# zichunhao/lgn-autoencoder

Measured on AMD Instinct MI355X. Metric: jets/sec fwd+bwd, 30-particle maxdim=2 bs=512, higher is better.
Workload: dtype f64

## Files before the change

### lgn-autoencoder_amd/csrc/level.hpp

```cpp
#pragma once
#include "common.hpp"

namespace lgn {

constexpr int LVL_DEC_PAIRWISE = 2;
constexpr int LVL_LEVEL_V2 = 4;
constexpr int LVL_MLP_V1 = 8;
constexpr int LVL_MOMENTS_V1 = 16;
constexpr int LVL_MLP_BWD1 = 1024;
constexpr int LVL_MLP_FULLTILE = 2048;
constexpr int LVL_MOMENTS_SPLIT = 512;
constexpr int LVL_LIVE_SCALARS = 4096;
constexpr int LVL_BWD_ORDERED = 64;
int level_flags_from_env();

template <typename T>
struct LevelArgs {
  int B, N, C, CO;
  const T* s_in;
  const T* v_in;
  const T* p;
  const uint8_t* mask;
  const T *ra, *rb, *rc, *w0, *b0, *w1, *b1;
  const T *wm0, *wm1;
  T* ag0;
  T* ag1;
  T* s_out;
// ... 5 lines not shown
  T* z1 = nullptr;
  size_t z1n = 0;
  T* z2 = nullptr;
  size_t z2n = 0;
  const T* loss_wo1 = nullptr;
  const T* loss_target = nullptr;
  T loss_scale = T(1);
  int loss_real = 0;
  T loss_jscale = T(0);
  T* loss_recon = nullptr;
  T* loss_part = nullptr;
  T* loss_gv = nullptr;
  T* loss_wpart = nullptr;
  int flags = 0;
  int dead_scalars = 0;
};

template <typename T>
struct LevelBwdArgs {
  int B, N, C, CO;
  const T *s_in, *v_in, *p;
  const uint8_t* mask;
  const T *ra, *rb, *rc, *w0, *b0, *w1, *b1;
  const T *wm0, *wm1;
  const T *ag0, *ag1;
  const T* g_s_out;
  const T* g_v_out;
  T* g_ag;
  T* g_s_in;
  T* g_v_in;
  T* g_p;
  T* part_mix;
  T* part_rad;
  T* part_in0 = nullptr;
  int flags = 0;
  int dead_scalars = 0;
};

__host__ __device__ constexpr int node_stride(int C) { return 10 * C + 4; }

__host__ __device__ constexpr int rad_partial_size(int C, bool dec) {
  return dec ? 2 * C : (2 * 4 * C * NB + 8 * C);
}

inline int level_jet_split(int B, int N) {
  const int groups = (N + 3) / 4;
  int s = 1;
  while (s * 2 <= groups && B * s * 2 <= 512) s *= 2;
  return s;
}

// ... 2 lines not shown
```

### lgn-autoencoder_amd/csrc/level_bwd.hip

```cpp
#include <stdlib.h>

#include "level_dev.hpp"
#include <type_traits>
#include "ops.hpp"
#include "tail_dev.hpp"

namespace lgn {

template <int C> struct GA {
  static constexpr int A3 = 0, A4 = 2 * C, A1 = 4 * C, A2 = 12 * C, SIZE = 20 * C;
};

template <typename T, int C>
__global__ __launch_bounds__(BLOCK) void level_bwd_mix_kernel(LevelBwdArgs<T> a) {
  constexpr int IT = 32;
  constexpr int K = 5 * C;
  constexpr int XS = K * 10;
  const int N = a.N, B = a.B, CO = a.CO;
  const int b = blockIdx.x, tile = blockIdx.y, tid = threadIdx.x;
  const int GS = CO * 10;

  extern __shared__ __align__(16) unsigned char smem_raw[];
  T* sm = reinterpret_cast<T*>(smem_raw);
  T* wm = sm;
// ... 340 lines not shown
  return 0;
}

int level_bwd_nodes2_dispatch(const LevelBwdArgs<double>& a, int decoder, hipStream_t stream);
int level_bwd_rad2_dispatch(const LevelBwdArgs<double>& a, hipStream_t stream);

int level_bwd3_dispatch(const LevelBwdArgs<double>& a, int decoder, hipStream_t stream);
int level_bwd_dec_sep_dispatch(const LevelBwdArgs<double>& a, hipStream_t stream);
int level_bwd_sweep_enc_dispatch(const LevelBwdArgs<double>& a, hipStream_t stream);
static bool dec_pairwise(int flags) { return (flags & LVL_DEC_PAIRWISE) != 0; }
bool level_bwd3_fits(int N);

static bool use_v3(int N, int flags) { return !(flags & LVL_LEVEL_V2) && level_bwd3_fits(N); }

bool level_bwd_carries_input(int N, int flags) { return use_v3(N, flags); }

void level_bwd_partial_rows(int B, int N, int decoder, int flags, int* rows_mix, int* rows_rad) {
  const int tiles = cdiv(N, 32);
  if (use_v3(N, flags)) {
    const int split = (decoder && !dec_pairwise(flags)) ? 1 : level_jet_split(B, N);
    *rows_mix = B * split;
    *rows_rad = B * split;
    return;
  }
  *rows_mix = B * tiles;
  if (decoder && dec_pairwise(flags)) {
    *rows_rad = B * tiles;
  } else {
    *rows_rad = B;
  }
}

template <typename T, int C, bool DEC>
static int launch_level_bwd(const LevelBwdArgs<T>& a, hipStream_t stream) {
  using L = Carve<C, DEC>;
  const int N = a.N, CO = a.CO, tiles = cdiv(N, 32);
  int rc;
  if (use_v3(N, a.flags)) return level_bwd3_dispatch(a, DEC, stream);
  {
    auto kern = level_bwd_mix_kernel<T, C>;
    size_t smem = sizeof(T) * (4 * CO * 5 * C + 32 * (5 * C * 10) + 32 * CO * 10);
    if ((rc = ensure_smem(kern, smem, "level_bwd_mix"))) return rc;
    hipLaunchKernelGGL(kern, dim3(a.B, tiles), dim3(BLOCK), smem, stream, a);
    LGN_CHECK_LAUNCH();
  }
  if constexpr (DEC && std::is_same<T, double>::value) {
    if (!dec_pairwise(a.flags)) return level_bwd_dec_sep_dispatch(a, stream);
  }
  if constexpr (!DEC && std::is_same<T, double>::value) {
    if (!(a.flags & LVL_LEVEL_V2)) return level_bwd_sweep_enc_dispatch(a, stream);
  }
  if ((rc = level_bwd_nodes2_dispatch(a, DEC, stream))) return rc;
  if (DEC) {
// ... 110 lines not shown
```

### lgn-autoencoder_amd/csrc/level_bwd3.hip

```cpp
#include "pair_dev.hpp"
#include "ops.hpp"
#include "wave_sum.hpp"

namespace lgn {

namespace {
LGN_STAMP_DECL
}
LGN_STAMP_READER(lgn_debug_stamps_bwd3)

template <int C, bool DEC, int NWV = 4>
struct Bwd3 {
  static constexpr int BLK = 64 * NWV;
  static constexpr int NG = (C + 3) / 4;
  static constexpr int NS = node_stride(C);
  static constexpr int PS = DEC ? 8 : 4;
  static constexpr int TRSZ = DEC ? NWV * 64 : NWV * pair_scratch(NG);
  static constexpr int MIXP = BLK / (5 * C) < 16 ? BLK / (5 * C) : 16;
  __host__ __device__ static size_t scratch(int N, int CO) {
    size_t p1 = (size_t)N * 10 * CO + 4 * CO * 5 * C + (size_t)N * 20 * C;
    const size_t red = (size_t)MIXP * CO * 5 * C * 4;
    if (red > p1) p1 = red;
    return p1 > (size_t)TRSZ ? p1 : (size_t)TRSZ;
  }
// ... 19 lines not shown
  const int nlo = min(N, 4 * glo), nhi = min(N, 4 * ghi);
  const size_t prow = (size_t)b * gridDim.y + blockIdx.y;

  extern __shared__ __align__(16) unsigned char smem_raw[];
  double* nd = reinterpret_cast<double*>(smem_raw);
  double* ga = nd + ((N * NS + 1) & ~1);
  double* gd = ga + N * G::SIZE;
  double* pj = gd + N * 10 * C;
  double* tr = pj + N * PS;
  double* go = tr;
  double* wm = go + N * 10 * CO;
  double* agl = wm + 4 * CO * K;
  double* sm = tr + F::scratch(N, CO);
  uint8_t* mk = reinterpret_cast<uint8_t*>(sm + F::SEPSZ);

  STAMP(0);
  {
    const size_t plo = (size_t)B * N * CO, pa = (size_t)B * N * 2 * C;
    JetRegs<double> jr;
    load_jet_issue<double, C, DEC>(a.s_in, a.v_in, a.p, a.mask, B, N, b, jr);
    const int eg = tid < N * CO ? tid : 0, ea_ = tid < N * 2 * C ? tid : 0, ew = tid < 2 * CO * K ? tid : 0;
    const size_t ig = (size_t)b * N * CO + eg, ia = (size_t)b * N * 2 * C + ea_;
    double rg[10], ra[10];
    if constexpr (!NOS) {
      rg[0] = a.g_s_out[ig];
      rg[1] = a.g_s_out[plo + ig];
      ra[0] = a.ag0[ia];
      ra[1] = a.ag0[pa + ia];
    }
#pragma unroll
    for (int m = 0; m < 4; ++m) {
      rg[2 + m] = a.g_v_out[ig * 4 + m];
      rg[6 + m] = a.g_v_out[plo * 4 + ig * 4 + m];
      ra[2 + m] = a.ag1[ia * 4 + m];
      ra[6 + m] = a.ag1[(pa + ia) * 4 + m];
    }
    const double w0v = a.wm0[ew], w1v = a.wm1[ew];
    load_jet_commit<double, C, DEC>(a.s_in, a.v_in, a.p, a.mask, B, N, b, jr, nd, pj, mk);
    if (tid < N * CO) {
#pragma unroll
      for (int m = NOS ? 2 : 0; m < 10; ++m) go[tid * 10 + m] = rg[m];
    }
    if (tid < N * 2 * C) {
#pragma unroll
      for (int m = NOS ? 2 : 0; m < 10; ++m) agl[tid * 10 + m] = ra[m];
    }
    if (tid < 2 * CO * K) {
      wm[tid] = w0v;
      wm[2 * CO * K + tid] = w1v;
    }
    for (int e = tid + BLK; e < 2 * CO * K; e += BLK) {
      wm[e] = a.wm0[e];
      wm[2 * CO * K + e] = a.wm1[e];
    }
    for (int e = tid + BLK; e < N * CO; e += BLK) {
      const size_t idx = (size_t)b * N * CO + e;
      double* g = go + e * 10;
      if constexpr (!NOS) {
        g[0] = a.g_s_out[idx];
        g[1] = a.g_s_out[plo + idx];
      }
#pragma unroll
      for (int m = 0; m < 4; ++m) {
        g[2 + m] = a.g_v_out[idx * 4 + m];
        g[6 + m] = a.g_v_out[plo * 4 + idx * 4 + m];
      }
    }
    for (int e = tid + BLK; e < N * 2 * C; e += BLK) {
      const size_t ea = (size_t)b * N * 2 * C + e;
      double* x = agl + e * 10;
      if constexpr (!NOS) {
        x[0] = a.ag0[ea];
        x[1] = a.ag0[pa + ea];
      }
#pragma unroll
      for (int m = 0; m < 4; ++m) {
        x[2 + m] = a.ag1[ea * 4 + m];
        x[6 + m] = a.ag1[(pa + ea) * 4 + m];
      }
    }
  }
  __syncthreads();
  STAMP(1);

  {
    const int half = tid >= BLK / 2;
    for (int e = half ? tid - BLK / 2 : tid; e < N * C; e += BLK / 2) {
      const int n = e / C, c = e - n * C;
      const double* w0r = wm + c;
      const double* w1r = wm + 2 * CO * K + c;
      if (half == 0) {
        cx<double> gx0[2] = {{0, 0}, {0, 0}}, gx1[2][4] = {{{0, 0}, {0, 0}, {0, 0}, {0, 0}}, {{0, 0}, {0, 0}, {0, 0}, {0, 0}}};
        for (int o = 0; o < CO; ++o) {
          const double* g = go + (n * CO + o) * 10;
          cx<double> gv[4];
#pragma unroll
          for (int m = 0; m < 4; ++m) gv[m] = {g[2 + m], g[6 + m]};
// ... 131 lines not shown
    STAMP(51);
    for (int ex = tid; ex < 4 * OK; ex += BLK) {
      const int e = ex >> 2, x = ex & 3;
      if (NOS && x < 2) continue;
      double v = red[ex];
#pragma unroll
      for (int pp = 1; pp < NPART; ++pp) v += red[pp * OK * 4 + ex];
      part[x * OK + e] = v;
    }
  }

  if constexpr (DEC && SEP) {
    STAMP(3);
    __syncthreads();
    STAMP(4);
    if (tid < 64) {
      const int k = tid & 7, part = tid >> 3;
      double mean = 0.0;
      for (int n = part; n < N; n += 8) mean += pj[n * 8 + k];
      mean += shfl_xor(mean, 8);
      mean += shfl_xor(mean, 16);
      mean += shfl_xor(mean, 32);
      if (part == 0) sm[k] = mean / N;
    }
    __syncthreads();
    for (int e = tid; e < N * 8; e += BLK) pj[e] -= sm[e & 7];
    __syncthreads();
#define LGN_PUT(k, val)                                       \
  do {                                                        \
    if ((k) < 16) a0[(k) < 16 ? (k) : 0] += (val);                                        \
    else if ((k) < 32) a1[(k) >= 16 && (k) < 32 ? (k) - 16 : 0] += (val);                 \
    else if ((k) < 44) a2[(k) >= 32 && (k) < 44 ? (k) - 32 : 0] += (val);                 \
    else a3[(k) >= 44 ? (k) - 44 : 0] += (val);                                           \
  } while (0)
    for (int c = wave; c < C; c += NWV) {
      double a0[16], a1[16], a2[12], a3[8];
#pragma unroll
      for (int k = 0; k < 16; ++k) a0[k] = a1[k] = 0.0;
#pragma unroll
      for (int k = 0; k < 12; ++k) a2[k] = 0.0;
#pragma unroll
      for (int k = 0; k < 8; ++k) a3[k] = 0.0;
// ... 529 lines not shown
    rad_rows_store(tr, wave, lane, T);
    __syncthreads();
    const int wq = __builtin_amdgcn_readfirstlane(wave);
    if (wq < 4) rad_rows_sum<C, NWV, WaveSum::Pairwise, true>(tr, part, lane, wq);
  }
  STAMP(10);
}

bool level_bwd3_fits(int N) { return N <= 40; }

template <int C, bool DEC, bool SEP, int NWV, bool NOS>
static int launch_bwd3_w(const LevelBwdArgs<double>& a, int split, hipStream_t stream) {
  size_t smem = Bwd3<C, DEC, NWV>::smem(a.N, a.CO);
  LGN_CHECK_ARG(smem <= 160 * 1024, "level_bwd: N=%d C=%d needs %zu B of LDS", a.N, a.C, smem);
  LGN_CHECK_ARG(a.CO <= 8, "level_bwd: C_out=%d unsupported (1..8)", a.CO);
  auto kern = level_bwd3_kernel<C, DEC, SEP, NWV, false, NOS>;
  if constexpr (!DEC && C <= 4) {
    if (split == 1 && !(a.flags & LVL_BWD_ORDERED)) kern = level_bwd3_kernel<C, DEC, SEP, NWV, true, NOS>;
  }
  if (smem > 64 * 1024) (void)hipFuncSetAttribute(reinterpret_cast<const void*>(kern), hipFuncAttributeMaxDynamicSharedMemorySize, (int)smem);
  hipLaunchKernelGGL(kern, dim3(a.B, split), dim3(64 * NWV), smem, stream, a);
  LGN_CHECK_LAUNCH();
  return 0;
}
template <int C, bool DEC, bool SEP>
static int launch_bwd3(const LevelBwdArgs<double>& a, hipStream_t stream) {
  const int split = SEP ? 1 : level_jet_split(a.B, a.N);
  return a.dead_scalars ? launch_bwd3_w<C, DEC, SEP, 4, true>(a, split, stream) : launch_bwd3_w<C, DEC, SEP, 4, false>(a, split, stream);
}

// ... 19 lines not shown
```

### lgn-autoencoder_amd/csrc/level_dev.hpp

```cpp
#pragma once
#include "level.hpp"

namespace lgn {

template <int C, bool DEC>
struct Carve {
  static constexpr int R = 4 * C;
  static constexpr int NS = node_stride(C);
  static constexpr int PS = DEC ? 8 : 4;
  static constexpr int RA = 0, RB = NB, RC = 2 * NB;
  static constexpr int RW = 3 * NB;
  static constexpr int RBIAS = RW + NB * R;
  static constexpr int RAD_SIZE = RBIAS + R;
  __host__ __device__ static constexpr int even(int x) { return (x + 1) & ~1; }
};

template <typename T>
struct JetRegs {
  T s[2], v[8], p[2];
  uint8_t m;
};
template <typename T, int C, bool DEC>
__device__ __forceinline__ void load_jet_issue(const T* __restrict__ s_in, const T* __restrict__ v_in, const T* __restrict__ p,
                                               const uint8_t* __restrict__ mask, int B, int N, int b, JetRegs<T>& r) {
// ... 100 lines not shown
  }
  return g;
}

template <typename T>
__device__ __forceinline__ cx<T> bil2(const cx<T> (&a)[4], const cx<T> (&b)[4]) {
  cx<T> r = cmul(a[0], b[0]);
  cfma(r, a[1], b[3]);
  cx<T> t = cmul(a[2], b[2]);
  r.r -= t.r;
  r.i -= t.i;
  cfma(r, a[3], b[1]);
  return r;
}

template <typename T>
__device__ __forceinline__ void metric_perm(const cx<T> (&x)[4], cx<T> (&y)[4]) {
  y[0] = x[0];
  y[1] = x[3];
  y[2] = {-x[2].r, -x[2].i};
  y[3] = x[1];
}

__device__ __forceinline__ void rcp5(const double (&u)[5], double (&r)[5]) {
  const double p1 = u[0] * u[1], p2 = p1 * u[2], p3 = p2 * u[3], p4 = p3 * u[4];
  if (__builtin_expect(!(p4 < 0x1p+1000), 0)) {
#pragma unroll
    for (int s = 0; s < 5; ++s) r[s] = 1.0 / u[s];
    return;
  }
// ... 14 lines not shown
```

### lgn-autoencoder_amd/csrc/level_fwd2.hip

```cpp
#include "level_dev.hpp"
#include "net_dev.hpp"
#include "ops.hpp"
#include "wave_sum.hpp"

namespace lgn {

LGN_STAMP_DECL
LGN_STAMP_READER(lgn_debug_stamps_fwd2)

template <int C, bool DEC>
struct Fwd2 {
  static constexpr int NG = (C + 3) / 4;
  static constexpr int NS = node_stride(C);
  static constexpr int PS = DEC ? 8 : 4;
  static constexpr int AGS = 20 * C;
  static constexpr int A3 = 0, A4 = 2 * C, A1 = 4 * C, A2 = 12 * C;
};

template <int C, bool DEC, bool SEP, bool TRAIN, bool NOS>
__global__ __launch_bounds__(2 * BLOCK) void level_fwd2_kernel(LevelArgs<double> a, int chunk) {
  using F = Fwd2<C, DEC>;
  constexpr int NG = F::NG;
  const int N = a.N, B = a.B, CO = a.CO;
  const int b = blockIdx.x, tid = threadIdx.x, lane = tid & 63, wave = tid >> 6;
// ... 99 lines not shown
      const double* bb = (q >> 1) ? a.b1 : a.b0;
      bias[g][q] = ch < C ? (DEC ? bb[ch] : bb[2 * ch + (q & 1)]) : 0.0;
    }
  }
  __syncthreads();
  STAMP(1);

  if constexpr (DEC && SEP) {
    if (tid < 64) {
      const int k = tid & 7, part = tid >> 3;
      double mean = 0.0;
      for (int n = part; n < N; n += 8) mean += pj[n * 8 + k];
      mean += shfl_xor(mean, 8);
      mean += shfl_xor(mean, 16);
      mean += shfl_xor(mean, 32);
      if (part == 0) sums[k] = mean / N;
    }
    __syncthreads();
    for (int e = tid; e < N * 8; e += nthr) pj[e] -= sums[e & 7];
    __syncthreads();
#define LGN_PUT(k, val)                                           \
  do {                                                            \
    if ((k) < 12) a0[(k) < 12 ? (k) : 0] += (val);                \
    else a1[(k) >= 12 ? (k) - 12 : 0] += (val);                   \
  } while (0)
    for (int c = wave; c < C; c += nw) {
      double a0[12], a1[8];
#pragma unroll
      for (int k = 0; k < 12; ++k) a0[k] = 0.0;
#pragma unroll
      for (int k = 0; k < 8; ++k) a1[k] = 0.0;
// ... 12 lines not shown
        for (int m = 0; m < 4; ++m) {
          LGN_PUT(2 + 2 * m, v[m].r);  LGN_PUT(3 + 2 * m, v[m].i);
          const cx<double> sp = cmul(sn, pc[m]);
          LGN_PUT(10 + 2 * m, sp.r);  LGN_PUT(11 + 2 * m, sp.i);
        }
        if constexpr (!NOS) {
          const cx<double> vp = bil2(v, pc);
          LGN_PUT(18, vp.r);  LGN_PUT(19, vp.i);
        }
      }
      wave_sum_store<12>(a0, sums + c * 20, lane);
      wave_sum_store<8>(a1, sums + c * 20 + 12, lane);
    }
#undef LGN_PUT
    __syncthreads();
  }

  const int ngroups = (N + 3) >> 2, gper = (ngroups + (int)gridDim.y - 1) / (int)gridDim.y;
  const int rlo = min(N, 4 * (int)blockIdx.y * gper), rhi = min(N, rlo + 4 * gper);
  auto catmix = [&](int c0, int c1) {
    constexpr int K = 5 * C;
    const int nr = c1 - c0;
    const size_t plo = (size_t)B * N * CO;
    const int vfirst = NOS ? tid : lane + 64 * (wave - 1), vstep = NOS ? nthr : 64 * (nw - 1);
    if (!NOS && wave == 0) {
      for (int rl = lane; rl < nr; rl += 64) {
        const int r = c0 + rl;
        const double* st = agl + rl * F::AGS;
        const double* ni = nd + r * F::NS;
        cx<double> x[K];
// ... 45 lines not shown
          cx<double> acc = {0, 0};
#pragma unroll
          for (int k = 0; k < K; ++k) cfma(acc, cx<double>{wr[k], wi[k]}, x[k]);
          const size_t e = ((size_t)b * N + r) * CO + o;
          a.v_out[e * 4 + m] = acc.r;
          a.v_out[plo * 4 + e * 4 + m] = acc.i;
        }
      }
    }
    };
  for (int c0 = rlo; c0 < rhi; c0 += chunk) {
  const int c1 = min(rhi, c0 + chunk);
  if constexpr (DEC && SEP) {
    for (int e = tid; e < (c1 - c0) * C; e += nthr) {
      const int rl = e / C, c = e - rl * C, n = c0 + rl;
      const double* sm = sums + c * 20;
      const double* pn = pj + n * 8;
      const cx<double> R0 = {a.b0[c], a.b0[c]}, R1 = {a.b1[c], a.b1[c]};
      const cx<double> e0 = {R0.r - R0.i, R0.r + R0.i};
      const cx<double> S = {sm[0], sm[1]};
      cx<double> VS[4], pc[4];
#pragma unroll
      for (int m = 0; m < 4; ++m) {
        VS[m] = {sm[2 + 2 * m], sm[3 + 2 * m]};
        pc[m] = {pn[m], pn[4 + m]};
      }
      double* st = agl + rl * F::AGS;
      if constexpr (!NOS) {
        const cx<double> a4 = cmul(S, e0);
        cx<double> t = bil2(VS, pc);
        t.r -= sm[18];  t.i -= sm[19];
        cx<double> a3 = cmul(R1, t);
        st[F::A3 + 2 * c] = 0.5 * a3.r;  st[F::A3 + 2 * c + 1] = 0.5 * a3.i;
        st[F::A4 + 2 * c] = a4.r;        st[F::A4 + 2 * c + 1] = a4.i;
      }
#pragma unroll
      for (int m = 0; m < 4; ++m) {
        const cx<double> a1 = cmul(VS[m], e0);
        cx<double> u = cmul(pc[m], S);
        u.r -= sm[10 + 2 * m];  u.i -= sm[11 + 2 * m];
        const cx<double> a2 = cmul(R1, u);
        st[F::A1 + (c * 4 + m) * 2] = a1.r;  st[F::A1 + (c * 4 + m) * 2 + 1] = a1.i;
        st[F::A2 + (c * 4 + m) * 2] = a2.r;  st[F::A2 + (c * 4 + m) * 2 + 1] = a2.i;
      }
    }
  } else {
  const int ngr = (c1 - c0 + 3) >> 2;
  const int rs = (!DEC && nw == 4 && ngr >= 1 && ngr <= 2 && chunk >= 16) ? 4 / ngr : 1;
  const int rpart = rs > 1 ? wave % rs : 0, ntl = (N + 3) >> 2;
  auto row_group = [&](const int rg, const int jlo, const int jhi, const int slab) __attribute__((always_inline)) {
    const int i0 = rg * 4;
    const int i = i0 + ti;
    const bool iok = i < N;
    const int ii = iok ? i : N - 1;
    double pi[F::PS];
#pragma unroll
    for (int m = 0; m < F::PS; ++m) pi[m] = pj[ii * F::PS + m];
    const bool mi = DEC ? false : (mk[ii] != 0);
// ... 156 lines not shown
  }
  if (rs > 1) {
    __syncthreads();
    const int tot = 4 * ngr * F::AGS;
    for (int e = tid; e < tot; e += nthr) {
      if (NOS && e % F::AGS < F::A1) continue;
      double v = agl[e];
      for (int pp = 1; pp < rs; ++pp) v += agl[pp * tot + e];
      agl[e] = v;
    }
  }
  }
  __syncthreads();
  STAMP(20);

  if constexpr (TRAIN) {
    const size_t pl0 = (size_t)B * N * 2 * C;
    if constexpr (!NOS) {
      for (int e = tid; e < (c1 - c0) * 2 * C; e += nthr) {
        const int n = e / (2 * C), r = e - n * 2 * C, blk = r / C, ch = r - blk * C;
        const double* st = agl + n * F::AGS + (blk ? F::A4 : F::A3) + 2 * ch;
        const size_t ge = ((size_t)b * N + c0) * 2 * C + e;
        a.ag0[ge] = st[0];
        a.ag0[pl0 + ge] = st[1];
      }
    }
    for (int e = tid; e < (c1 - c0) * 2 * C * 4; e += nthr) {
      const int n = e / (8 * C), r = e - n * 8 * C, blk = r / (4 * C), cm = r - blk * 4 * C;
      const double* st = agl + n * F::AGS + (blk ? F::A2 : F::A1) + 2 * cm;
      const size_t ge = ((size_t)b * N + c0) * 8 * C + e;
      a.ag1[ge] = st[0];
// ... 24 lines not shown
  const size_t row = sizeof(double) * F::AGS, budget1 = 160 * 1024, budget2 = wide ? budget1 : 78 * 1024;
  const int full = (a.N + 15) & ~15;
  int chunk = full;
  if (fixed + full * row > budget2) {
    const size_t room = fixed + 16 * row <= budget2 ? budget2 - fixed : (fixed < budget1 ? budget1 - fixed : 0);
    chunk = (int)(room / row) & ~15;
    if (chunk > full) chunk = full;
    if (chunk < 16) chunk = 16;
  }
  size_t smem = fixed + chunk * row;
  if (a.loss_wo1) {
    LGN_CHECK_ARG(DEC && SEP && a.N <= 40 && !wide && a.loss_target && a.loss_recon && a.loss_part && (!TRAIN || (a.loss_gv && a.loss_wpart)),
                  "level_fwd: the loss rides on the separable decoder forward of jets of <= 40 particles only");
    if (smem < dec_out_loss_bytes(a.N, a.CO)) smem = dec_out_loss_bytes(a.N, a.CO);
  }
  LGN_CHECK_ARG(smem <= 160 * 1024, "level_fwd: N=%d C=%d needs %zu B of LDS (> 160 KiB)", a.N, a.C, smem);
  auto kern = level_fwd2_kernel<C, DEC, SEP, TRAIN, NOS>;
  if (smem > 64 * 1024) {
    hipError_t e = hipFuncSetAttribute(reinterpret_cast<const void*>(kern), hipFuncAttributeMaxDynamicSharedMemorySize, (int)smem);
    if (e != hipSuccess) { set_error("hipFuncSetAttribute: %s", hipGetErrorString(e)); return (int)e; }
  }
  const int nthreads = wide ? 2 * BLOCK : BLOCK;
  const int split = (SEP || a.N > 40) ? 1 : level_jet_split(a.B, a.N);
  hipLaunchKernelGGL(kern, dim3(a.B, split), dim3(nthreads), smem, stream, a, chunk);
  LGN_CHECK_LAUNCH();
  return 0;
}

bool level_fwd_carries_loss(int N, int flags) { return N <= 40 && !(flags & LVL_DEC_PAIRWISE); }

// ... 34 lines not shown
```

### lgn-autoencoder_amd/csrc/ops.hpp

```cpp
#pragma once
#include <cstdlib>
#include <vector>
#include "level.hpp"

namespace lgn {

template <typename T> int level_fwd_dispatch(const LevelArgs<T>&, int decoder, hipStream_t);
int level_fwd_eval(const LevelArgs<double>&, int decoder, hipStream_t);
template <typename T> int level_bwd_dispatch(const LevelBwdArgs<T>&, int decoder, hipStream_t);
template <typename T> int reduce_partials(const T* part, int rows, int n, T* out, int accumulate, hipStream_t);
template <typename T> int reduce_partials_strided(const T* part, int rows, int stride, int col0, int n, T* out, hipStream_t);
constexpr int RED_MAX_SEG = 64;
template <typename T> struct RedSeg { const T* part; int rows, stride, col0, n; T* out; };
template <typename T> struct RedJob {
  int nseg;
  RedSeg<T> seg[RED_MAX_SEG];
  int tile0[RED_MAX_SEG + 1];
  void add(const T* part, int rows, int stride, int col0, int n, T* out) { seg[nseg++] = RedSeg<T>{part, rows, stride, col0, n, out}; }
};
template <typename T> int reduce_segments(RedJob<T>& job, hipStream_t);
template <typename T>
int rad_finalize(const T* tot, int C, const T* ra, const T* rb, const T* rc, const T* w0, const T* w1, T* g_a, T* g_b, T* g_c,
                 T* g_w0, T* g_b0, T* g_w1, T* g_b1, hipStream_t);
struct RadFinJob {
// ... 8 lines not shown
  long* step_dev;
  double lambda, lr, beta1, beta2, eps;
  int do_adam;
  const double* loss_part;
  int nB;
  double* loss_out;
  int reduce_only;
  unsigned long long* counters;
  int opt_form = 0;
  int kind = 0;
  double l2 = 0.0, alpha = 0.0, mu = 0.0;
};
int step_tail(const std::vector<RedSeg<double>>& segs, const RadFinJob& fin, const StepTailArgs& ta, hipStream_t st);
void level_bwd_partial_rows(int B, int N, int decoder, int flags, int* rows_mix, int* rows_rad);
bool level_bwd_carries_input(int N, int flags);
bool level_fwd_carries_loss(int N, int flags);

constexpr int MLP_MAX_LIN = 8;
template <typename T>
struct MlpArgs {
  int M;
  int C;
  int H;
  int nlin;
  const T* w[MLP_MAX_LIN];
  const T* b[MLP_MAX_LIN];
  const T* s_in;
  T* s_out;
  const T* g_out;
  T* g_in;
// ... 146 lines not shown
```

### lgn-autoencoder_amd/csrc/step.hip

```cpp
#include <stdlib.h>

#include <algorithm>
#include <mutex>
#include <vector>

#include "net.hpp"
#include "../../include/lgn_amd.h"

namespace lgn {
namespace {

struct Bump {
  double* base;
  size_t off = 0;
  double* take(size_t n) {
    n = (n + 15) & ~size_t(15);
    double* p = base ? base + off : nullptr;
    off += n;
    return p;
  }
};

struct NetBuf {
  double *s[5], *v[5], *smix[4], *ag0[4], *ag1[4];
  double* hsave[4];
};

struct Work {
  NetBuf enc, dec;
  double *lat_s, *lat_v, *pdec, *g_lat_s, *g_lat_v, *g_p;
  double *gs[2], *gv[2], *gsmix, *g_ag, *zeros_s;
  double *parts;
  size_t parts_size;
  double* tot[2][4];
  int* idx;
  size_t total;
  double* tail_cnt;
  double* zero0() const { return tail_cnt < zeros_s ? tail_cnt : zeros_s; }
  size_t zero_doubles;
};
// ... 120 lines not shown
  const int Nd = dec_nodes(d), Nmax = d.N > Nd ? d.N : Nd;
  const size_t BNe = (size_t)d.B * d.N, BNd = (size_t)d.B * Nd, BN = (size_t)d.B * Nmax;
  const int L = d.n_levels;
  int cmax = 0;
  for (int l = 0; l <= L; ++l) cmax = cmax > d.enc_channels[l] ? cmax : d.enc_channels[l], cmax = cmax > d.dec_channels[l] ? cmax : d.dec_channels[l];
  auto net = [&](NetBuf& n, const int* ch, bool dec) {
    const size_t BN = dec ? BNd : BNe;
    for (int l = 0; l <= L; ++l) {
      n.s[l] = b.take(2 * BN * ch[l]);
      n.v[l] = b.take(8 * BN * ch[l]);
    }
    for (int l = 0; l < L; ++l) {
      n.smix[l] = b.take(2 * BN * ch[l + 1]);
      n.ag0[l] = b.take(4 * BN * ch[l]);
      n.ag1[l] = b.take(16 * BN * ch[l]);
      const size_t hs = l + 1 < L && BN <= mlp_save_max_rows()
                            ? mlp_saved_doubles((int)BN, d.mlp_hidden_mul * 2 * ch[l + 1], d.mlp_nlin) : 0;
      n.hsave[l] = hs ? b.take(hs) : nullptr;
    }
  };
  net(w.enc, d.enc_channels, false);
  net(w.dec, d.dec_channels, true);
  const int Ts = d.tau_s, Tv = d.tau_v, PB = pool_blocks(d.latent_pool);
  w.lat_s = b.take((size_t)2 * d.B * PB * Ts);
  w.lat_v = b.take((size_t)2 * d.B * PB * Tv * 4);
  w.g_lat_v = b.take((size_t)2 * d.B * PB * Tv * 4);
  w.pdec = b.take(8 * BN);
  for (int q = 0; q < 2; ++q) {
    w.gs[q] = b.take(2 * BN * cmax);
    w.gv[q] = b.take(8 * BN * cmax);
// ... 62 lines not shown
    auto p = [&](int slot) { return P + off[slot]; };
    LevelArgs<double> a{d.B, d.N, ch[l], ch[l + 1], n.s[l], n.v[l], pos, mask,
                        p(S.rad(dec, l, 0)), p(S.rad(dec, l, 1)), p(S.rad(dec, l, 2)), p(S.rad(dec, l, 3)), p(S.rad(dec, l, 4)),
                        p(S.rad(dec, l, 5)), p(S.rad(dec, l, 6)), p(S.mix(dec, l, 0)), p(S.mix(dec, l, 1)),
                        n.ag0[l], n.ag1[l], n.smix[l], n.v[l + 1]};
    if (l == 0 && !dec && in0) {
      a.in_w0 = in0->w0; a.in_w1 = in0->w1; a.in_s = n.s[0]; a.in_v = n.v[0];
      a.z1 = in0->z1; a.z1n = in0->z1n; a.z2 = in0->z2; a.z2n = in0->z2n;
    }
    if (l + 1 == d.n_levels && dec && loss) {
      a.loss_wo1 = loss->wo1; a.loss_target = loss->target; a.loss_scale = loss->scale; a.loss_real = loss->method;
      a.loss_jscale = loss->jscale; a.loss_recon = loss->recon;
      a.loss_part = loss->loss_part; a.loss_gv = loss->g_v; a.loss_wpart = loss->wpart;
    }
    a.flags = d.flags;
    const bool no_mlp = l + 1 == d.n_levels && (!last_scalars || (eval && dec));
    a.dead_scalars = no_mlp && !(d.flags & LVL_LIVE_SCALARS);
    LGN_TRY(eval ? level_fwd_eval(a, dec, st) : level_fwd_dispatch<double>(a, dec, st));
    if (no_mlp) break;
    MlpArgs<double> m = level_mlp_args(d, dec, l, P, off);
    m.s_in = n.smix[l]; m.s_out = n.s[l + 1];
    m.h_saved = n.hsave[l]; m.h_rows = mlp_saved_rows(m.M);
    LGN_TRY(mlp_dispatch<double>(m, false, st));
  }
  return 0;
}

int levels_bwd(const lgn_net_desc& d, bool dec, const int* ch, const double* P, double* G, const int64_t* off, const NetBuf& n,
               const double* pos, const uint8_t* mask, Work& w, Deferred& dq, RadFinJob& fin, int& cur, bool has_s_grad,
               hipStream_t st, bool* in0_done = nullptr) {
// ... 19 lines not shown
    level_bwd_partial_rows(d.B, d.N, dec, d.flags, &rm, &rr);
    const int nmix = 4 * CO * 5 * C, nrad = rad_partial_size(C, dec);
    DQ_NEW(part_mix, (size_t)rm * nmix);
    DQ_NEW(part_rad, (size_t)rr * nrad);
    const int nxt = cur ^ 1;
    LevelBwdArgs<double> a{d.B, d.N, C, CO, n.s[l], n.v[l], pos, mask,
                           p(S.rad(dec, l, 0)), p(S.rad(dec, l, 1)), p(S.rad(dec, l, 2)), p(S.rad(dec, l, 3)), p(S.rad(dec, l, 4)),
                           p(S.rad(dec, l, 5)), p(S.rad(dec, l, 6)), p(S.mix(dec, l, 0)), p(S.mix(dec, l, 1)), n.ag0[l], n.ag1[l],
                           g_smix, w.gv[cur], w.g_ag, w.gs[nxt], w.gv[nxt], dec ? w.g_p : nullptr, part_mix, part_rad};
    const bool dead_s = !has_s_grad && !(d.flags & LVL_LIVE_SCALARS);
    a.dead_scalars = dead_s;
    const bool carry_in0 = !dec && l == 0 && in0_done && level_bwd_carries_input(d.N, d.flags);
    const RowLayout rin = enc_input_rows(1, C);
    if (carry_in0) { DQ_TAKE(a.part_in0, (size_t)rm * rin.width); }
    a.flags = d.flags;
    LGN_TRY(level_bwd_dispatch<double>(a, dec, st));
    if (carry_in0) {
      rin.add(dq, a.part_in0, rm, G, off);
      *in0_done = true;
    }
    if (dead_s) dq.add(nullptr, 0, 0, 0, nmix / 2, g(S.mix(dec, l, 0)));
    else dq.add(part_mix, rm, nmix, 0, nmix / 2, g(S.mix(dec, l, 0)));
    dq.add(part_mix, rm, nmix, nmix / 2, nmix / 2, g(S.mix(dec, l, 1)));
    if (dec) {
      dq.add(part_rad, rr, nrad, 0, C, g(S.rad(dec, l, 4)));
      dq.add(part_rad, rr, nrad, C, C, g(S.rad(dec, l, 6)));
    } else {
      double* tot = w.tot[0][l];
      dq.add(part_rad, rr, nrad, 0, nrad, tot);
      fin.it[fin.n++] = RadFinJob::Item{tot, C, p(S.rad(dec, l, 0)), p(S.rad(dec, l, 1)), p(S.rad(dec, l, 2)), p(S.rad(dec, l, 3)),
// ... 574 lines not shown
  size_t total;
};
NetAct carve_act(const lgn_net_desc& d, bool dec, double* base) {
  NetAct a{};
  Bump b{base};
  const size_t BN = (size_t)d.B * d.N;
  const int* ch = dec ? d.dec_channels : d.enc_channels;
  for (int l = 0; l <= d.n_levels; ++l) {
    a.n.s[l] = b.take(2 * BN * ch[l]);
    a.n.v[l] = b.take(8 * BN * ch[l]);
  }
  for (int l = 0; l < d.n_levels; ++l) {
    a.n.smix[l] = b.take(2 * BN * ch[l + 1]);
    a.n.ag0[l] = b.take(4 * BN * ch[l]);
    a.n.ag1[l] = b.take(16 * BN * ch[l]);
    const size_t hs = BN <= mlp_save_max_rows()
                          ? mlp_saved_doubles((int)BN, d.mlp_hidden_mul * 2 * ch[l + 1], d.mlp_nlin) : 0;
    a.n.hsave[l] = hs ? b.take(hs) : nullptr;
  }
  if (dec) a.pdec = b.take(8 * BN);
  else a.idx = reinterpret_cast<int*>(b.take(((size_t)d.B * 2 * (d.tau_s + d.tau_v) * 2 + 1) / 2 + 8));
  a.total = b.off;
  return a;
}

struct NetScratch {
  Work w;
  size_t total;
};
NetScratch carve_scratch(const lgn_net_desc& d, bool dec, double* base) {
// ... 591 lines not shown
```

### lgn-autoencoder_amd/lgn/_native.py

```python
from __future__ import annotations

import ctypes as C
import os
from typing import Optional, Sequence

import torch

_HERE = os.path.dirname(os.path.abspath(__file__))
LIB_PATH = os.environ.get("LGN_AMD_LIB") or os.path.join(_HERE, "_lib", "liblgn_amd.so")
ABI_VERSION = 19
FINALIZE_SCRATCH = 2048
FINALIZE_OPT_SCRATCH = 4096

_lib: Optional[C.CDLL] = None

_vp, _i, _ip = C.c_void_p, C.c_int, C.POINTER(C.c_int)

_SIGNATURES = {
    "lgn_level_fwd_f64": [_i] * 5 + [_vp] * 18,
    "lgn_level_bwd_partial_rows": [_i, _i, _i, _ip, _ip],
    "lgn_level_rad_partial_len": [_i, _i],
    "lgn_level_jet_split": [_i, _i],
    "lgn_cg_product_fwd_f64": [_i] * 8 + [_vp] * 7,
    "lgn_cg_product_bwd_f64": [_i] * 8 + [_vp] * 9,
# ... 70 lines not shown
                ("mlp_nlin", C.c_int), ("tau_v_in", C.c_int),
                ("enc_tables", _tp * 4), ("dec_tables", _tp * 4),
                ("enc_Q", C.c_int * 5), ("enc_qs", C.c_int * 5), ("enc_qv", C.c_int * 5),
                ("dec_Q", C.c_int * 5), ("dec_qs", C.c_int * 5), ("dec_qv", C.c_int * 5), ("flags", C.c_int),
                ("activation", C.c_int), ("n_in_scalars", C.c_int), ("latent_pool", C.c_int), ("dec_N", C.c_int),
                ("get_real", C.c_int), ("jet_loss_scale", C.c_double)]

    def __init__(self, *a, **kw):
        super().__init__(*a, **kw)
        self.flags = net_flags()


NET_NO_STATIC = 1
_NET_FLAG_ENV = {"LGN_AMD_NO_STATIC": 1, "LGN_AMD_DEC_PAIRWISE": 2, "LGN_AMD_LEVEL_V2": 4, "LGN_AMD_MLP_V1": 8,
                 "LGN_AMD_MOMENTS_V1": 16, "LGN_AMD_BWD_ORDERED": 64, "LGN_AMD_LIVE_SCALARS": 4096, "LGN_AMD_SPLIT_TAIL": 128, "LGN_AMD_DEC_UNFUSED": 256, "LGN_AMD_MOMENTS_SPLIT": 512,
                 "LGN_AMD_MLP_BWD1": 1024, "LGN_AMD_MLP_FULLTILE": 2048}
ACTIVATIONS = {"leakyrelu": 0, "relu": 1, "elu": 2, "sigmoid": 3, "logsigmoid": 4, "atan": 5}


def activation_id(name: str) -> int:
    try:
        return ACTIVATIONS[name.lower()]
    except KeyError:
        raise ValueError(f"Activation function {name} not implemented!") from None


def net_flags() -> int:
    return sum(bit for name, bit in _NET_FLAG_ENV.items() if os.environ.get(name, "") == "1")


class LossDesc(C.Structure):
# ... 372 lines not shown
```

Measured before the change: 1.116 million.

## Rebuild decoder aggregate in backward from stored per-jet sums instead of storing it

In training, the separable decoder forward now writes only the small per-jet sums and particle means rather than the full per-particle aggregate tensors ag0/ag1. The backward kernel reloads these sums and recomputes the aggregate rows in LDS through a shared helper that both passes use. This trades a large global write and read of aggregate data for a little extra arithmetic in the backward. A new env flag restores the old store path.

```diff
diff --git a/lgn-autoencoder_amd/csrc/level.hpp b/lgn-autoencoder_amd/csrc/level.hpp
--- a/lgn-autoencoder_amd/csrc/level.hpp
+++ b/lgn-autoencoder_amd/csrc/level.hpp
@@ -11,6 +11,7 @@
 constexpr int LVL_MLP_FULLTILE = 2048;
 constexpr int LVL_MOMENTS_SPLIT = 512;
 constexpr int LVL_LIVE_SCALARS = 4096;
+constexpr int LVL_DEC_STORE_AG = 16384;
 constexpr int LVL_BWD_ORDERED = 64;
 int level_flags_from_env();
 
@@ -46,7 +47,9 @@
   T* loss_wpart = nullptr;
   int flags = 0;
   int dead_scalars = 0;
+  T* sep_sums = nullptr;
 };
+constexpr int sep_sums_doubles(int C) { return 20 * C + 8; }
 
 template <typename T>
 struct LevelBwdArgs {
@@ -67,6 +70,7 @@
   T* part_in0 = nullptr;
   int flags = 0;
   int dead_scalars = 0;
+  const T* sep_sums = nullptr;
 };
 
 __host__ __device__ constexpr int node_stride(int C) { return 10 * C + 4; }
diff --git a/lgn-autoencoder_amd/csrc/level_bwd.hip b/lgn-autoencoder_amd/csrc/level_bwd.hip
--- a/lgn-autoencoder_amd/csrc/level_bwd.hip
+++ b/lgn-autoencoder_amd/csrc/level_bwd.hip
@@ -378,6 +378,7 @@
 static bool use_v3(int N, int flags) { return !(flags & LVL_LEVEL_V2) && level_bwd3_fits(N); }
 
 bool level_bwd_carries_input(int N, int flags) { return use_v3(N, flags); }
+bool level_dec_rebuilds(int N, int flags) { return use_v3(N, flags) && !(flags & (LVL_DEC_PAIRWISE | LVL_DEC_STORE_AG)); }
 
 void level_bwd_partial_rows(int B, int N, int decoder, int flags, int* rows_mix, int* rows_rad) {
   const int tiles = cdiv(N, 32);
@@ -401,6 +402,7 @@
   const int N = a.N, CO = a.CO, tiles = cdiv(N, 32);
   int rc;
   if (use_v3(N, a.flags)) return level_bwd3_dispatch(a, DEC, stream);
+  LGN_CHECK_ARG(!a.sep_sums, "level_bwd: N=%d: this form of the backward reads the stored aggregate", N);
   {
     auto kern = level_bwd_mix_kernel<T, C>;
     size_t smem = sizeof(T) * (4 * CO * 5 * C + 32 * (5 * C * 10) + 32 * CO * 10);
diff --git a/lgn-autoencoder_amd/csrc/level_bwd3.hip b/lgn-autoencoder_amd/csrc/level_bwd3.hip
--- a/lgn-autoencoder_amd/csrc/level_bwd3.hip
+++ b/lgn-autoencoder_amd/csrc/level_bwd3.hip
@@ -57,6 +57,8 @@
   double* sm = tr + F::scratch(N, CO);
   uint8_t* mk = reinterpret_cast<uint8_t*>(sm + F::SEPSZ);
 
+  bool rebuild = false;
+  if constexpr (DEC && SEP) rebuild = a.sep_sums != nullptr;
   STAMP(0);
   {
     const size_t plo = (size_t)B * N * CO, pa = (size_t)B * N * 2 * C;
@@ -64,19 +66,29 @@
     load_jet_issue<double, C, DEC>(a.s_in, a.v_in, a.p, a.mask, B, N, b, jr);
     const int eg = tid < N * CO ? tid : 0, ea_ = tid < N * 2 * C ? tid : 0, ew = tid < 2 * CO * K ? tid : 0;
     const size_t ig = (size_t)b * N * CO + eg, ia = (size_t)b * N * 2 * C + ea_;
-    double rg[10], ra[10];
+    double rg[10], ra[10], fs = 0.0;
     if constexpr (!NOS) {
       rg[0] = a.g_s_out[ig];
       rg[1] = a.g_s_out[plo + ig];
-      ra[0] = a.ag0[ia];
-      ra[1] = a.ag0[pa + ia];
     }
 #pragma unroll
     for (int m = 0; m < 4; ++m) {
       rg[2 + m] = a.g_v_out[ig * 4 + m];
       rg[6 + m] = a.g_v_out[plo * 4 + ig * 4 + m];
-      ra[2 + m] = a.ag1[ia * 4 + m];
-      ra[6 + m] = a.ag1[(pa + ia) * 4 + m];
+    }
+    if (!rebuild) {
+      if constexpr (!NOS) {
+        ra[0] = a.ag0[ia];
+        ra[1] = a.ag0[pa + ia];
+      }
+#pragma unroll
+      for (int m = 0; m < 4; ++m) {
+        ra[2 + m] = a.ag1[ia * 4 + m];
+        ra[6 + m] = a.ag1[(pa + ia) * 4 + m];
+      }
+    } else if constexpr (DEC && SEP) {
+      static_assert(sep_sums_doubles(C) <= BLK && sep_sums_doubles(C) <= F::SEPSZ, "the forward's sums are one item per thread, kept in sm");
+      fs = a.sep_sums[(size_t)b * sep_sums_doubles(C) + (tid < sep_sums_doubles(C) ? tid : 0)];
     }
     const double w0v = a.wm0[ew], w1v = a.wm1[ew];
     load_jet_commit<double, C, DEC>(a.s_in, a.v_in, a.p, a.mask, B, N, b, jr, nd, pj, mk);
@@ -84,10 +96,11 @@
 #pragma unroll
       for (int m = NOS ? 2 : 0; m < 10; ++m) go[tid * 10 + m] = rg[m];
     }
-    if (tid < N * 2 * C) {
+    if (!rebuild && tid < N * 2 * C) {
 #pragma unroll
       for (int m = NOS ? 2 : 0; m < 10; ++m) agl[tid * 10 + m] = ra[m];
     }
+    if (rebuild && tid < sep_sums_doubles(C)) sm[tid] = fs;
     if (tid < 2 * CO * K) {
       wm[tid] = w0v;
       wm[2 * CO * K + tid] = w1v;
@@ -109,7 +122,7 @@
         g[6 + m] = a.g_v_out[plo * 4 + idx * 4 + m];
       }
     }
-    for (int e = tid + BLK; e < N * 2 * C; e += BLK) {
+    for (int e = tid + BLK; !rebuild && e < N * 2 * C; e += BLK) {
       const size_t ea = (size_t)b * N * 2 * C + e;
       double* x = agl + e * 10;
       if constexpr (!NOS) {
@@ -124,6 +137,28 @@
     }
   }
   __syncthreads();
+  if constexpr (DEC && SEP) {
+    if (rebuild) {
+      for (int e = tid; e < N * 8; e += BLK) pj[e] -= sm[20 * C + (e & 7)];
+      __syncthreads();
+      for (int e = tid; e < N * C; e += BLK) {
+        const int n = e / C, c = e - n * C;
+        const SepRow row = dec_sep_row<NOS>(sm + c * 20, pj + n * 8, a.b0[c], a.b1[c]);
+        double* x0 = agl + (n * 2 * C + c) * 10;
+        double* x1 = agl + (n * 2 * C + C + c) * 10;
+        if constexpr (!NOS) {
+          x0[0] = row.a3h.r;  x0[1] = row.a3h.i;
+          x1[0] = row.a4.r;   x1[1] = row.a4.i;
+        }
+#pragma unroll
+        for (int m = 0; m < 4; ++m) {
+          x0[2 + m] = row.a1[m].r;  x0[6 + m] = row.a1[m].i;
+          x1[2 + m] = row.a2[m].r;  x1[6 + m] = row.a2[m].i;
+        }
+      }
+      __syncthreads();
+    }
+  }
   STAMP(1);
 
   {
@@ -285,18 +320,20 @@
     STAMP(3);
     __syncthreads();
     STAMP(4);
-    if (tid < 64) {
-      const int k = tid & 7, part = tid >> 3;
-      double mean = 0.0;
-      for (int n = part; n < N; n += 8) mean += pj[n * 8 + k];
-      mean += shfl_xor(mean, 8);
-      mean += shfl_xor(mean, 16);
-      mean += shfl_xor(mean, 32);
-      if (part == 0) sm[k] = mean / N;
-    }
-    __syncthreads();
-    for (int e = tid; e < N * 8; e += BLK) pj[e] -= sm[e & 7];
-    __syncthreads();
+    if (!rebuild) {
+      if (tid < 64) {
+        const int k = tid & 7, part = tid >> 3;
+        double mean = 0.0;
+        for (int n = part; n < N; n += 8) mean += pj[n * 8 + k];
+        mean += shfl_xor(mean, 8);
+        mean += shfl_xor(mean, 16);
+        mean += shfl_xor(mean, 32);
+        if (part == 0) sm[k] = mean / N;
+      }
+      __syncthreads();
+      for (int e = tid; e < N * 8; e += BLK) pj[e] -= sm[e & 7];
+      __syncthreads();
+    }
 #define LGN_PUT(k, val)                                       \
   do {                                                        \
     if ((k) < 16) a0[(k) < 16 ? (k) : 0] += (val);                                        \
@@ -856,6 +893,7 @@
   size_t smem = Bwd3<C, DEC, NWV>::smem(a.N, a.CO);
   LGN_CHECK_ARG(smem <= 160 * 1024, "level_bwd: N=%d C=%d needs %zu B of LDS", a.N, a.C, smem);
   LGN_CHECK_ARG(a.CO <= 8, "level_bwd: C_out=%d unsupported (1..8)", a.CO);
+  LGN_CHECK_ARG(!a.sep_sums || (DEC && SEP), "level_bwd: only the separable decoder backward rebuilds the aggregate from jet sums");
   auto kern = level_bwd3_kernel<C, DEC, SEP, NWV, false, NOS>;
   if constexpr (!DEC && C <= 4) {
     if (split == 1 && !(a.flags & LVL_BWD_ORDERED)) kern = level_bwd3_kernel<C, DEC, SEP, NWV, true, NOS>;
diff --git a/lgn-autoencoder_amd/csrc/level_dev.hpp b/lgn-autoencoder_amd/csrc/level_dev.hpp
--- a/lgn-autoencoder_amd/csrc/level_dev.hpp
+++ b/lgn-autoencoder_amd/csrc/level_dev.hpp
@@ -138,6 +138,52 @@
   return r;
 }
 
+struct SepRow {
+  cx<double> a3h, a4, a1[4], a2[4];
+};
+template <bool NOS>
+__device__ __forceinline__ SepRow dec_sep_row(const double* sm, const double* pn, double b0, double b1) {
+#pragma clang fp contract(off)
+  const cx<double> e0 = {b0 - b0, b0 + b0};
+  const cx<double> S = {sm[0], sm[1]};
+  cx<double> VS[4], pc[4];
+#pragma unroll
+  for (int m = 0; m < 4; ++m) {
+    VS[m] = {sm[2 + 2 * m], sm[3 + 2 * m]};
+    pc[m] = {pn[m], pn[4 + m]};
+  }
+  SepRow o;
+  if constexpr (!NOS) {
+    o.a4.r = __builtin_fma(S.r, e0.r, -(S.i * e0.i));
+    o.a4.i = __builtin_fma(S.r, e0.i, S.i * e0.r);
+    cx<double> t, u;
+    t.r = __builtin_fma(VS[0].r, pc[0].r, -(VS[0].i * pc[0].i));
+    t.i = __builtin_fma(VS[0].i, pc[0].r, VS[0].r * pc[0].i);
+    cfma(t, VS[1], pc[3]);
+    u.r = __builtin_fma(VS[2].r, pc[2].r, -(VS[2].i * pc[2].i));
+    u.i = __builtin_fma(VS[2].i, pc[2].r, VS[2].r * pc[2].i);
+    t.r -= u.r;  t.i -= u.i;
+    cfma(t, VS[3], pc[1]);
+    t.r -= sm[18];  t.i -= sm[19];
+    const double w = b1 * t.i;
+    o.a3h.r = 0.5 * __builtin_fma(b1, t.r, -w);
+    o.a3h.i = 0.5 * __builtin_fma(b1, t.r, w);
+  }
+#pragma unroll
+  for (int m = 0; m < 4; ++m) {
+    o.a1[m].r = __builtin_fma(VS[m].r, e0.r, -(VS[m].i * e0.i));
+    o.a1[m].i = __builtin_fma(VS[m].r, e0.i, VS[m].i * e0.r);
+    cx<double> u;
+    u.r = __builtin_fma(pc[m].r, S.r, -(pc[m].i * S.i));
+    u.i = __builtin_fma(pc[m].r, S.i, pc[m].i * S.r);
+    u.r -= sm[10 + 2 * m];  u.i -= sm[11 + 2 * m];
+    const double w = b1 * u.i;
+    o.a2[m].r = __builtin_fma(b1, u.r, -w);
+    o.a2[m].i = __builtin_fma(b1, u.r, w);
+  }
+  return o;
+}
+
 template <typename T>
 __device__ __forceinline__ void metric_perm(const cx<T> (&x)[4], cx<T> (&y)[4]) {
   y[0] = x[0];
diff --git a/lgn-autoencoder_amd/csrc/level_fwd2.hip b/lgn-autoencoder_amd/csrc/level_fwd2.hip
--- a/lgn-autoencoder_amd/csrc/level_fwd2.hip
+++ b/lgn-autoencoder_amd/csrc/level_fwd2.hip
@@ -137,7 +137,13 @@
       mean += shfl_xor(mean, 8);
       mean += shfl_xor(mean, 16);
       mean += shfl_xor(mean, 32);
-      if (part == 0) sums[k] = mean / N;
+      if (part == 0) {
+        const double mu = mean / N;
+        sums[k] = mu;
+        if constexpr (TRAIN) {
+          if (a.sep_sums) a.sep_sums[(size_t)b * sep_sums_doubles(C) + 20 * C + k] = mu;
+        }
+      }
     }
     __syncthreads();
     for (int e = tid; e < N * 8; e += nthr) pj[e] -= sums[e & 7];
@@ -180,6 +186,10 @@
     }
 #undef LGN_PUT
     __syncthreads();
+    if constexpr (TRAIN) {
+      if (a.sep_sums)
+        for (int e = tid; e < 20 * C; e += nthr) a.sep_sums[(size_t)b * sep_sums_doubles(C) + e] = sums[e];
+    }
   }
 
   const int ngroups = (N + 3) >> 2, gper = (ngroups + (int)gridDim.y - 1) / (int)gridDim.y;
@@ -255,34 +265,16 @@
   if constexpr (DEC && SEP) {
     for (int e = tid; e < (c1 - c0) * C; e += nthr) {
       const int rl = e / C, c = e - rl * C, n = c0 + rl;
-      const double* sm = sums + c * 20;
-      const double* pn = pj + n * 8;
-      const cx<double> R0 = {a.b0[c], a.b0[c]}, R1 = {a.b1[c], a.b1[c]};
-      const cx<double> e0 = {R0.r - R0.i, R0.r + R0.i};
-      const cx<double> S = {sm[0], sm[1]};
-      cx<double> VS[4], pc[4];
-#pragma unroll
-      for (int m = 0; m < 4; ++m) {
-        VS[m] = {sm[2 + 2 * m], sm[3 + 2 * m]};
-        pc[m] = {pn[m], pn[4 + m]};
-      }
+      const SepRow row = dec_sep_row<NOS>(sums + c * 20, pj + n * 8, a.b0[c], a.b1[c]);
       double* st = agl + rl * F::AGS;
       if constexpr (!NOS) {
-        const cx<double> a4 = cmul(S, e0);
-        cx<double> t = bil2(VS, pc);
-        t.r -= sm[18];  t.i -= sm[19];
-        cx<double> a3 = cmul(R1, t);
-        st[F::A3 + 2 * c] = 0.5 * a3.r;  st[F::A3 + 2 * c + 1] = 0.5 * a3.i;
-        st[F::A4 + 2 * c] = a4.r;        st[F::A4 + 2 * c + 1] = a4.i;
+        st[F::A3 + 2 * c] = row.a3h.r;  st[F::A3 + 2 * c + 1] = row.a3h.i;
+        st[F::A4 + 2 * c] = row.a4.r;   st[F::A4 + 2 * c + 1] = row.a4.i;
       }
 #pragma unroll
       for (int m = 0; m < 4; ++m) {
-        const cx<double> a1 = cmul(VS[m], e0);
-        cx<double> u = cmul(pc[m], S);
-        u.r -= sm[10 + 2 * m];  u.i -= sm[11 + 2 * m];
-        const cx<double> a2 = cmul(R1, u);
-        st[F::A1 + (c * 4 + m) * 2] = a1.r;  st[F::A1 + (c * 4 + m) * 2 + 1] = a1.i;
-        st[F::A2 + (c * 4 + m) * 2] = a2.r;  st[F::A2 + (c * 4 + m) * 2 + 1] = a2.i;
+        st[F::A1 + (c * 4 + m) * 2] = row.a1[m].r;  st[F::A1 + (c * 4 + m) * 2 + 1] = row.a1[m].i;
+        st[F::A2 + (c * 4 + m) * 2] = row.a2[m].r;  st[F::A2 + (c * 4 + m) * 2 + 1] = row.a2[m].i;
       }
     }
   } else {
@@ -469,7 +461,7 @@
   __syncthreads();
   STAMP(20);
 
-  if constexpr (TRAIN) {
+  if (TRAIN && !(DEC && SEP && a.sep_sums)) {
     const size_t pl0 = (size_t)B * N * 2 * C;
     if constexpr (!NOS) {
       for (int e = tid; e < (c1 - c0) * 2 * C; e += nthr) {
@@ -524,6 +516,8 @@
                   "level_fwd: the loss rides on the separable decoder forward of jets of <= 40 particles only");
     if (smem < dec_out_loss_bytes(a.N, a.CO)) smem = dec_out_loss_bytes(a.N, a.CO);
   }
+  LGN_CHECK_ARG(!a.sep_sums || (DEC && SEP && TRAIN && a.N <= 40),
+                "level_fwd: only the separable decoder forward of a training step (N <= 40) leaves jet sums instead of the aggregate");
   LGN_CHECK_ARG(smem <= 160 * 1024, "level_fwd: N=%d C=%d needs %zu B of LDS (> 160 KiB)", a.N, a.C, smem);
   auto kern = level_fwd2_kernel<C, DEC, SEP, TRAIN, NOS>;
   if (smem > 64 * 1024) {
diff --git a/lgn-autoencoder_amd/csrc/ops.hpp b/lgn-autoencoder_amd/csrc/ops.hpp
--- a/lgn-autoencoder_amd/csrc/ops.hpp
+++ b/lgn-autoencoder_amd/csrc/ops.hpp
@@ -46,6 +46,7 @@
 int step_tail(const std::vector<RedSeg<double>>& segs, const RadFinJob& fin, const StepTailArgs& ta, hipStream_t st);
 void level_bwd_partial_rows(int B, int N, int decoder, int flags, int* rows_mix, int* rows_rad);
 bool level_bwd_carries_input(int N, int flags);
+bool level_dec_rebuilds(int N, int flags);
 bool level_fwd_carries_loss(int N, int flags);
 
 constexpr int MLP_MAX_LIN = 8;
diff --git a/lgn-autoencoder_amd/csrc/step.hip b/lgn-autoencoder_amd/csrc/step.hip
--- a/lgn-autoencoder_amd/csrc/step.hip
+++ b/lgn-autoencoder_amd/csrc/step.hip
@@ -24,6 +24,7 @@
 struct NetBuf {
   double *s[5], *v[5], *smix[4], *ag0[4], *ag1[4];
   double* hsave[4];
+  double* sep[4];
 };
 
 struct Work {
@@ -174,6 +175,7 @@
       n.smix[l] = b.take(2 * BN * ch[l + 1]);
       n.ag0[l] = b.take(4 * BN * ch[l]);
       n.ag1[l] = b.take(16 * BN * ch[l]);
+      n.sep[l] = dec ? b.take((size_t)d.B * sep_sums_doubles(ch[l])) : nullptr;
       const size_t hs = l + 1 < L && BN <= mlp_save_max_rows()
                             ? mlp_saved_doubles((int)BN, d.mlp_hidden_mul * 2 * ch[l + 1], d.mlp_nlin) : 0;
       n.hsave[l] = hs ? b.take(hs) : nullptr;
@@ -266,6 +268,7 @@
       a.loss_part = loss->loss_part; a.loss_gv = loss->g_v; a.loss_wpart = loss->wpart;
     }
     a.flags = d.flags;
+    if (dec && !eval && level_dec_rebuilds(d.N, d.flags)) a.sep_sums = n.sep[l];
     const bool no_mlp = l + 1 == d.n_levels && (!last_scalars || (eval && dec));
     a.dead_scalars = no_mlp && !(d.flags & LVL_LIVE_SCALARS);
     LGN_TRY(eval ? level_fwd_eval(a, dec, st) : level_fwd_dispatch<double>(a, dec, st));
@@ -315,6 +318,7 @@
     const RowLayout rin = enc_input_rows(1, C);
     if (carry_in0) { DQ_TAKE(a.part_in0, (size_t)rm * rin.width); }
     a.flags = d.flags;
+    if (dec && level_dec_rebuilds(d.N, d.flags)) a.sep_sums = n.sep[l];
     LGN_TRY(level_bwd_dispatch<double>(a, dec, st));
     if (carry_in0) {
       rin.add(dq, a.part_in0, rm, G, off);
@@ -919,6 +923,7 @@
     a.n.smix[l] = b.take(2 * BN * ch[l + 1]);
     a.n.ag0[l] = b.take(4 * BN * ch[l]);
     a.n.ag1[l] = b.take(16 * BN * ch[l]);
+    a.n.sep[l] = dec ? b.take((size_t)d.B * sep_sums_doubles(ch[l])) : nullptr;
     const size_t hs = BN <= mlp_save_max_rows()
                           ? mlp_saved_doubles((int)BN, d.mlp_hidden_mul * 2 * ch[l + 1], d.mlp_nlin) : 0;
     a.n.hsave[l] = hs ? b.take(hs) : nullptr;
diff --git a/lgn-autoencoder_amd/lgn/_native.py b/lgn-autoencoder_amd/lgn/_native.py
--- a/lgn-autoencoder_amd/lgn/_native.py
+++ b/lgn-autoencoder_amd/lgn/_native.py
@@ -108,7 +108,8 @@
 NET_NO_STATIC = 1
 _NET_FLAG_ENV = {"LGN_AMD_NO_STATIC": 1, "LGN_AMD_DEC_PAIRWISE": 2, "LGN_AMD_LEVEL_V2": 4, "LGN_AMD_MLP_V1": 8,
                  "LGN_AMD_MOMENTS_V1": 16, "LGN_AMD_BWD_ORDERED": 64, "LGN_AMD_LIVE_SCALARS": 4096, "LGN_AMD_SPLIT_TAIL": 128, "LGN_AMD_DEC_UNFUSED": 256, "LGN_AMD_MOMENTS_SPLIT": 512,
-                 "LGN_AMD_MLP_BWD1": 1024, "LGN_AMD_MLP_FULLTILE": 2048}
+                 "LGN_AMD_MLP_BWD1": 1024, "LGN_AMD_MLP_FULLTILE": 2048,
+                 "LGN_AMD_DEC_STORE_AG": 16384}
 ACTIVATIONS = {"leakyrelu": 0, "relu": 1, "elu": 2, "sigmoid": 3, "logsigmoid": 4, "atan": 5}
 
 
```

Result: faster. 1.134 million (median of 6 runs) (+1.6%).
